# kongzhecn/OMG

Measured on AMD Instinct MI355X. Metric: images/sec @ SDXL 1024^2 50-step, 2-concept mask fusion, higher is better.
Workload: dtype fp16 (storage and MFMA operands; fp32 accumulate; = the reference's own torch_dtype, inference_lora.py:153-159).  Measured tolerance per UNet forward at full size vs the fp32 oracle: rms 1.09e-3, max 4.9e-3 of O(1) outputs — the reference's own fp16 eager execution, emulated op by op in the oracle

## Files before the change

### omg_amd/csrc/misc.hip

```cpp
#include "common.h"
#include <string.h>

static thread_local char g_err[256] = "";
void omg_set_error(const char* msg) { strncpy(g_err, msg ? msg : "", sizeof(g_err) - 1); g_err[sizeof(g_err) - 1] = 0; }
extern "C" const char* omg_last_error(void) { return g_err; }
extern "C" int omg_abi_version(void) { return OMG_ABI_VERSION; }

namespace {

template <typename T, typename TI>
__global__ __launch_bounds__(256) void im2col_in_kernel(const TI* X, int B, int Cin, int H, int W, int KP, char* out) {
  const long npix = (long)B * H * W;
  for (long pix = (long)blockIdx.x * blockDim.x + threadIdx.x; pix < npix; pix += (long)gridDim.x * blockDim.x) {
    const int b = (int)(pix / (H * W)); const int rem = (int)(pix - (long)b * H * W);
    const int y = rem / W, x = rem - y * W;
    for (int c8 = 0; c8 < KP / 8; ++c8) {
      float f[8];
#pragma unroll
      for (int e = 0; e < 8; ++e) {
        const int k = c8 * 8 + e;
        const int tap = k / Cin, ci = k - tap * Cin;
        const int iy = y + tap / 3 - 1, ix = x + tap % 3 - 1;
        const bool ok = (tap < 9) && iy >= 0 && iy < H && ix >= 0 && ix < W;
        f[e] = ok ? (float)X[(((long)b * Cin + ci) * H + iy) * W + ix] : 0.f;
      }
      *(u32x4*)(out + (pix * KP + c8 * 8) * 2) = pack8<T>(f);
    }
  }
}

template <typename T>
__global__ __launch_bounds__(256) void conv_out_kernel(const char* X, int B, int H, int W, int Cin, const char* Wt,
                                                        const T* bias, int Cout, float* Y) {
  const int lane = threadIdx.x & 63, w = threadIdx.x >> 6;
  const long npix = (long)B * H * W;
  const int nvec = Cin / 8;
  const int K = 9 * Cin;
  for (long pix = (long)blockIdx.x * 4 + w; pix < npix; pix += (long)gridDim.x * 4) {
    const int b = (int)(pix / (H * W)); const int rem = (int)(pix - (long)b * H * W);
    const int y = rem / W, x = rem - y * W;
    float acc[8];
#pragma unroll
    for (int e = 0; e < 8; ++e) acc[e] = 0.f;
    for (int i = lane; i < 9 * nvec; i += 64) {
      const int tap = i / nvec, vec = i - tap * nvec;
      const int iy = y + tap / 3 - 1, ix = x + tap % 3 - 1;
      if (iy < 0 || iy >= H || ix < 0 || ix >= W) continue;
      float f[8];
      load8<T>(X + ((((long)b * H + iy) * W + ix) * Cin + vec * 8) * (long)sizeof(T), f);
#pragma unroll
      for (int co = 0; co < 8; ++co) {
        if (co < Cout) {
          float wv[8];
          load8<T>(Wt + ((long)co * K + tap * Cin + vec * 8) * (long)sizeof(T), wv);
#pragma unroll
          for (int e = 0; e < 8; ++e) acc[co] += f[e] * wv[e];
        }
      }
    }
#pragma unroll
    for (int co = 0; co < 8; ++co) {
#pragma unroll
      for (int off = 32; off > 0; off >>= 1) acc[co] += __shfl_xor(acc[co], off);
    }
    if (lane < Cout) {
      float v = 0.f;
#pragma unroll
      for (int co = 0; co < 8; ++co) if (co == lane) v = acc[co];
      Y[(((long)b * Cout + lane) * H + y) * W + x] = v + (bias ? (float)bias[lane] : 0.f);
    }
  }
}

template <typename T> struct Dot2;
template <> struct Dot2<f16> {
  typedef _Float16 v2 __attribute__((ext_vector_type(2)));
  static OMG_DEV float run(unsigned a, unsigned b, float c) { return __builtin_amdgcn_fdot2(__builtin_bit_cast(v2, a), __builtin_bit_cast(v2, b), c, false); }
};
template <> struct Dot2<bf16> {
  typedef __bf16 v2 __attribute__((ext_vector_type(2)));
  static OMG_DEV float run(unsigned a, unsigned b, float c) { return __builtin_amdgcn_fdot2_f32_bf16(__builtin_bit_cast(v2, a), __builtin_bit_cast(v2, b), c, false); }
};
template <typename T, int CO>
__global__ __launch_bounds__(256) void conv_out_pixel_kernel(const char* X, int B, int H, int W, int Cin, const char* Wt, const T* bias, float* Y) {
  const long npix = (long)B * H * W;
  const long pix = (long)blockIdx.x * 256 + threadIdx.x;
  const bool live = pix < npix;
  const long pc = live ? pix : npix - 1;
  const int b = (int)(pc / (H * W)); const int rem = (int)(pc - (long)b * H * W);
  const int y = rem / W, x = rem - y * W;
  const int nvec = Cin / 8;
  const long K2 = 9L * Cin * 2;
  float acc[CO];
#pragma unroll
  for (int co = 0; co < CO; ++co) acc[co] = 0.f;
  for (int tap = 0; tap < 9; ++tap) {
    const int iy = y + tap / 3 - 1, ix = x + tap % 3 - 1;
    const bool ok = ((unsigned)iy < (unsigned)H) & ((unsigned)ix < (unsigned)W);
    const u32x4* px = (const u32x4*)(X + ((((long)b * H + (ok ? iy : y)) * W + (ok ? ix : x)) * Cin) * 2);
    const char* wt = Wt + (long)tap * Cin * 2;
    for (int v0 = 0; v0 < nvec; v0 += 4) {
      u32x4 xv[4];
#pragma unroll
      for (int u = 0; u < 4; ++u) xv[u] = px[v0 + u];
#pragma unroll
      for (int u = 0; u < 4; ++u) {
        if (!ok) xv[u] = u32x4{0u, 0u, 0u, 0u};
#pragma unroll
        for (int co = 0; co < CO; ++co) {
          const u32x4 wv = *(const u32x4*)(wt + co * K2 + (v0 + u) * 16);
#pragma unroll
          for (int j = 0; j < 4; ++j) acc[co] = Dot2<T>::run(xv[u][j], wv[j], acc[co]);
        }
      }
    }
  }
  if (live) {
#pragma unroll
    for (int co = 0; co < CO; ++co) Y[(((long)b * CO + co) * H + y) * W + x] = acc[co] + (bias ? (float)bias[co] : 0.f);
  }
}

template <typename T>
__global__ void timestep_embedding_kernel(const float* t, int n, int dim, T* out, long ldo) {
  const int i = blockIdx.x;
  const int half = dim / 2;
  for (int j = threadIdx.x; j < dim; j += blockDim.x) {
    const int jj = j < half ? j : j - half;
    const float freq = expf(-9.210340371976184f * (float)jj / (float)half);
    const float a = t[i] * freq;
    out[(long)i * ldo + j] = (T)(j < half ? cosf(a) : sinf(a));
  }
}

template <typename T>
__global__ void silu_kernel(const T* x, T* y, long n) {
  for (long i = (long)blockIdx.x * blockDim.x + threadIdx.x; i < n; i += (long)gridDim.x * blockDim.x) y[i] = (T)silu_f((float)x[i]);
}

template <typename T>
__global__ void add_inplace_kernel(char* y, const char* a, long nvec) {
  for (long i = (long)blockIdx.x * blockDim.x + threadIdx.x; i < nvec; i += (long)gridDim.x * blockDim.x) {
    float f[8], g[8];
    unpack8<T>(*(const u32x4*)(y + i * 16), f);
    unpack8<T>(*(const u32x4*)(a + i * 16), g);
#pragma unroll
    for (int e = 0; e < 8; ++e) f[e] += g[e];
    *(u32x4*)(y + i * 16) = pack8<T>(f);
  }
}

template <typename T>
__global__ void copy2d_kernel(const T* src, long lds_, T* dst, long ldd, long rows, long cols) {
  const long n = rows * cols;
  for (long i = (long)blockIdx.x * blockDim.x + threadIdx.x; i < n; i += (long)gridDim.x * blockDim.x) {
    const long r = i / cols, c = i - r * cols;
    dst[r * ldd + c] = src[r * lds_ + c];
  }
}

__global__ void gather_step_kernel(const uint16_t* table, const int* step_idx, uint16_t* out, long n) {
  const long base = (long)(*step_idx) * n;
  for (long i = (long)blockIdx.x * blockDim.x + threadIdx.x; i < n; i += (long)gridDim.x * blockDim.x) out[i] = table[base + i];
}

struct StepP {
  int C, H, W, Hm, Wm, n_concepts, fuse;
  float gs;
  const float* noise;
  const float* region[OMG_MAX_CONCEPTS];
  const float* masks[OMG_MAX_CONCEPTS];
  const float* coef; int* step_idx; int advance;
  float* latents; int out_dtype; void* mi_next; float* fused_out;
};

__global__ __launch_bounds__(256) void step_kernel(StepP p) {
  const int HW = p.H * p.W;
  const int n = p.C * HW;
  const int step = *p.step_idx;
  const float cx = p.coef[step * 4 + 0], ce = p.coef[step * 4 + 1], cin = p.coef[step * 4 + 2];
  for (int i = blockIdx.x * blockDim.x + threadIdx.x; i < n; i += gridDim.x * blockDim.x) {
    const int c = i / HW; const int pix = i - c * HW;
    const int y = pix / p.W, x = pix - y * p.W;
    float unc0 = p.noise[0 * n + i], unc1 = p.noise[1 * n + i];
    float cnd0 = p.noise[2 * n + i], cnd1 = p.noise[3 * n + i];
    if (p.fuse) {
      const int my = (int)(((long)y * p.Hm) / p.H), mx = (int)(((long)x * p.Wm) / p.W);
      bool any = false;
      float add_u = 0.f, add_c = 0.f;
      for (int k = 0; k < p.n_concepts; ++k) {
        if (p.masks[k] == nullptr) continue;
        const bool on = p.masks[k][(long)my * p.Wm + mx] == 1.0f;
        if (on) {
          any = true;
          if (p.region[k]) { add_u += p.region[k][i]; add_c += p.region[k][n + i]; }
        }
      }
      unc1 = (any ? 0.f : unc1) + add_u;
      cnd1 = (any ? 0.f : cnd1) + add_c;
      if (p.fused_out) { p.fused_out[i] = unc1; p.fused_out[n + i] = cnd1; }
    }
    const float e0 = __fmaf_rn(p.gs, __fsub_rn(cnd0, unc0), unc0);
    const float e1 = __fmaf_rn(p.gs, __fsub_rn(cnd1, unc1), unc1);
    const float l0 = __fmaf_rn(ce, e0, __fmul_rn(cx, p.latents[i]));
    const float l1 = __fmaf_rn(ce, e1, __fmul_rn(cx, p.latents[n + i]));
    p.latents[i] = l0; p.latents[n + i] = l1;
    if (p.mi_next) {
      const float a0 = __fmul_rn(l0, cin), a1 = __fmul_rn(l1, cin);
      if (p.out_dtype == OMG_F16) {
        f16* o = (f16*)p.mi_next;
        o[i] = (f16)a0; o[n + i] = (f16)a1; o[2 * n + i] = (f16)a0; o[3 * n + i] = (f16)a1;
      } else if (p.out_dtype == OMG_BF16) {
        bf16* o = (bf16*)p.mi_next;
        o[i] = (bf16)a0; o[n + i] = (bf16)a1; o[2 * n + i] = (bf16)a0; o[3 * n + i] = (bf16)a1;
      } else {
        float* o = (float*)p.mi_next;
        o[i] = a0; o[n + i] = a1; o[2 * n + i] = a0; o[3 * n + i] = a1;
      }
    }
  }
}

__device__ __forceinline__ void step_fuse(const StepP& p, int i, int n, int HW, float& unc1, float& cnd1) {
  const int c = i / HW; const int pix = i - c * HW;
  const int y = pix / p.W, x = pix - y * p.W;
  const int my = (int)(((long)y * p.Hm) / p.H), mx = (int)(((long)x * p.Wm) / p.W);
  bool any = false;
  float add_u = 0.f, add_c = 0.f;
  for (int k = 0; k < p.n_concepts; ++k) {
    if (p.masks[k] == nullptr) continue;
    const bool on = p.masks[k][(long)my * p.Wm + mx] == 1.0f;
    if (on) {
      any = true;
      if (p.region[k]) { add_u += p.region[k][i]; add_c += p.region[k][n + i]; }
    }
  }
  unc1 = (any ? 0.f : unc1) + add_u;
  cnd1 = (any ? 0.f : cnd1) + add_c;
  if (p.fused_out) { p.fused_out[i] = unc1; p.fused_out[n + i] = cnd1; }
}

__device__ __forceinline__ void step_store_input(const StepP& p, int i, int n, float l0, float l1, float cin) {
  const float a0 = __fmul_rn(l0, cin), a1 = __fmul_rn(l1, cin);
  if (p.out_dtype == OMG_F16) {
    f16* o = (f16*)p.mi_next;
    o[i] = (f16)a0; o[n + i] = (f16)a1; o[2 * n + i] = (f16)a0; o[3 * n + i] = (f16)a1;
  } else if (p.out_dtype == OMG_BF16) {
    bf16* o = (bf16*)p.mi_next;
    o[i] = (bf16)a0; o[n + i] = (bf16)a1; o[2 * n + i] = (bf16)a0; o[3 * n + i] = (bf16)a1;
  } else {
    float* o = (float*)p.mi_next;
    o[i] = a0; o[n + i] = a1; o[2 * n + i] = a0; o[3 * n + i] = a1;
  }
}

__global__ __launch_bounds__(256) void step_ms_kernel(StepP p, const float* ms, float* hist) {
  const int HW = p.H * p.W;
  const int n = p.C * HW;
  const float* row = ms + (long)(*p.step_idx) * 8;
  const float a = row[0], b = row[1], cx = row[2], cm = row[3], cp = row[4], cin = row[5];
  const bool use_prev = cp != 0.f;
  for (int i = blockIdx.x * blockDim.x + threadIdx.x; i < n; i += gridDim.x * blockDim.x) {
    float unc0 = p.noise[0 * n + i], unc1 = p.noise[1 * n + i];
    float cnd0 = p.noise[2 * n + i], cnd1 = p.noise[3 * n + i];
    if (p.fuse) step_fuse(p, i, n, HW, unc1, cnd1);
    const float e0 = __fmaf_rn(p.gs, __fsub_rn(cnd0, unc0), unc0);
    const float e1 = __fmaf_rn(p.gs, __fsub_rn(cnd1, unc1), unc1);
    const float x0 = p.latents[i], x1 = p.latents[n + i];
    const float m0 = __fmaf_rn(b, e0, __fmul_rn(a, x0));
    const float m1 = __fmaf_rn(b, e1, __fmul_rn(a, x1));
    float l0 = __fmaf_rn(cm, m0, __fmul_rn(cx, x0));
    float l1 = __fmaf_rn(cm, m1, __fmul_rn(cx, x1));
    if (use_prev) {
      l0 = __fmaf_rn(cp, hist[i], l0);
      l1 = __fmaf_rn(cp, hist[n + i], l1);
    }
    hist[i] = m0; hist[n + i] = m1;
    p.latents[i] = l0; p.latents[n + i] = l1;
    if (p.mi_next) step_store_input(p, i, n, l0, l1, cin);
  }
}

__global__ __launch_bounds__(256) void step_noise_kernel(StepP p, const float* z, long zs) {
  const int HW = p.H * p.W;
  const int n = p.C * HW;
  const int step = *p.step_idx;
  const float cx = p.coef[step * 4 + 0], ce = p.coef[step * 4 + 1], cin = p.coef[step * 4 + 2], cz = p.coef[step * 4 + 3];
  const float* zt = z + (long)step * zs;
  const bool use_z = cz != 0.f;
  for (int i = blockIdx.x * blockDim.x + threadIdx.x; i < n; i += gridDim.x * blockDim.x) {
    float unc0 = p.noise[0 * n + i], unc1 = p.noise[1 * n + i];
    float cnd0 = p.noise[2 * n + i], cnd1 = p.noise[3 * n + i];
    if (p.fuse) step_fuse(p, i, n, HW, unc1, cnd1);
    const float e0 = __fmaf_rn(p.gs, __fsub_rn(cnd0, unc0), unc0);
    const float e1 = __fmaf_rn(p.gs, __fsub_rn(cnd1, unc1), unc1);
    float l0 = __fmaf_rn(ce, e0, __fmul_rn(cx, p.latents[i]));
    float l1 = __fmaf_rn(ce, e1, __fmul_rn(cx, p.latents[n + i]));
    if (use_z) {
      l0 = __fmaf_rn(cz, zt[i], l0);
      l1 = __fmaf_rn(cz, zt[n + i], l1);
    }
    p.latents[i] = l0; p.latents[n + i] = l1;
    if (p.mi_next) step_store_input(p, i, n, l0, l1, cin);
  }
}

__global__ void step_advance_kernel(int* step_idx) { *step_idx = *step_idx + 1; }

__global__ void scale_model_input_kernel(const float* latents, const float* cin, int n, int out_dtype, void* out) {
  const float c = *cin;
  for (int i = blockIdx.x * blockDim.x + threadIdx.x; i < 2 * n; i += gridDim.x * blockDim.x) {
    const float v = latents[i] * c;
    if (out_dtype == OMG_F16) { ((f16*)out)[i] = (f16)v; ((f16*)out)[2 * n + i] = (f16)v; }
    else if (out_dtype == OMG_BF16) { ((bf16*)out)[i] = (bf16)v; ((bf16*)out)[2 * n + i] = (bf16)v; }
    else { ((float*)out)[i] = v; ((float*)out)[2 * n + i] = v; }
  }
}

}

extern "C" int omg_conv_in(int dtype, const void* X, int x_is_f32, int B, int Cin, int H, int W, const void* Wt,
                           const void* bias, int Cout, void* workspace, void* Y, void* stream) {
  OMG_REQUIRE(dtype == OMG_F16 || dtype == OMG_BF16, "omg_conv_in: dtype");
  OMG_REQUIRE(X && Wt && Y && workspace && Cout % 8 == 0 && Cin > 0 && 9 * Cin <= 64, "omg_conv_in: args (9*Cin <= 64)");
  const long npix = (long)B * H * W;
  if (npix == 0) return OMG_OK;
  const int KP = 64;
  long blocks = (npix + 255) / 256; if (blocks > 8192) blocks = 8192;
  hipStream_t s = (hipStream_t)stream;
  if (dtype == OMG_F16) {
    if (x_is_f32) OMG_LAUNCH((im2col_in_kernel<f16, float>), dim3(blocks), dim3(256), 0, s, (const float*)X, B, Cin, H, W, KP, (char*)workspace);
    else OMG_LAUNCH((im2col_in_kernel<f16, f16>), dim3(blocks), dim3(256), 0, s, (const f16*)X, B, Cin, H, W, KP, (char*)workspace);
  } else {
    if (x_is_f32) OMG_LAUNCH((im2col_in_kernel<bf16, float>), dim3(blocks), dim3(256), 0, s, (const float*)X, B, Cin, H, W, KP, (char*)workspace);
    else OMG_LAUNCH((im2col_in_kernel<bf16, bf16>), dim3(blocks), dim3(256), 0, s, (const bf16*)X, B, Cin, H, W, KP, (char*)workspace);
  }
  int rc = omg_check_launch("im2col_in");
  if (rc) return rc;
  omg_gemm_args g{};
  g.dtype = dtype; g.M = (int)npix; g.N = Cout; g.K = KP;
  g.A = workspace; g.lda = KP; g.W = Wt; g.ldw = KP;
  g.groups = 1; g.rows_per_group = (int)npix; g.bias = bias; g.act = OMG_ACT_NONE; g.out_scale = 1.0f;
  g.C = Y; g.ldc = Cout;
  return omg_gemm(&g, stream);
}

template <typename T>
__global__ __launch_bounds__(256) void cast_f32_kernel(const char* X, float* Y, long n8) {
  for (long i = (long)blockIdx.x * 256 + threadIdx.x; i < n8; i += (long)gridDim.x * 256) {
    float f[8];
    load8<T>(X + i * 16, f);
    store8<float>((char*)(Y + i * 8), f);
  }
}

extern "C" int omg_cast_f32(int dtype, const void* X, float* Y, int64_t n, void* stream) {
  OMG_REQUIRE(dtype == OMG_F16 || dtype == OMG_BF16, "omg_cast_f32: dtype");
  OMG_REQUIRE(X && Y && n % 8 == 0, "omg_cast_f32: args");
  if (n == 0) return OMG_OK;
  long blocks = (n / 8 + 255) / 256; if (blocks > 16384) blocks = 16384;
  hipStream_t s = (hipStream_t)stream;
  if (dtype == OMG_F16) OMG_LAUNCH(cast_f32_kernel<f16>, dim3(blocks), dim3(256), 0, s, (const char*)X, Y, (long)(n / 8));
  else OMG_LAUNCH(cast_f32_kernel<bf16>, dim3(blocks), dim3(256), 0, s, (const char*)X, Y, (long)(n / 8));
  return omg_check_launch("cast_f32");
}

extern "C" int omg_conv_out(int dtype, const void* X, int B, int H, int W, int Cin, const void* Wt, const void* bias,
                            int Cout, float* Y, void* stream) {
  OMG_REQUIRE(dtype == OMG_F16 || dtype == OMG_BF16 || dtype == OMG_F32, "omg_conv_out: dtype");
  OMG_REQUIRE(X && Wt && Y && Cin % 8 == 0 && Cout >= 1 && Cout <= 8, "omg_conv_out: args");
  const long npix = (long)B * H * W;
  if (npix == 0) return OMG_OK;
  long blocks = (npix + 3) / 4; if (blocks > 8192) blocks = 8192;
  hipStream_t s = (hipStream_t)stream;
  if (dtype != OMG_F32 && Cout == 4 && Cin % 32 == 0 && (((uintptr_t)X | (uintptr_t)Wt) & 15) == 0) {
    const unsigned pb = (unsigned)((npix + 255) / 256);
    if (dtype == OMG_F16) OMG_LAUNCH((conv_out_pixel_kernel<f16, 4>), dim3(pb), dim3(256), 0, s, (const char*)X, B, H, W, Cin, (const char*)Wt, (const f16*)bias, Y);
    else OMG_LAUNCH((conv_out_pixel_kernel<bf16, 4>), dim3(pb), dim3(256), 0, s, (const char*)X, B, H, W, Cin, (const char*)Wt, (const bf16*)bias, Y);
    return omg_check_launch("conv_out_pixel");
  }
  if (dtype == OMG_F16) OMG_LAUNCH(conv_out_kernel<f16>, dim3(blocks), dim3(256), 0, s, (const char*)X, B, H, W, Cin, (const char*)Wt, (const f16*)bias, Cout, Y);
  else if (dtype == OMG_BF16) OMG_LAUNCH(conv_out_kernel<bf16>, dim3(blocks), dim3(256), 0, s, (const char*)X, B, H, W, Cin, (const char*)Wt, (const bf16*)bias, Cout, Y);
  else OMG_LAUNCH(conv_out_kernel<float>, dim3(blocks), dim3(256), 0, s, (const char*)X, B, H, W, Cin, (const char*)Wt, (const float*)bias, Cout, Y);
  return omg_check_launch("conv_out");
}

extern "C" int omg_timestep_embedding(int dtype, const float* t, int n, int dim, void* out, int64_t ldo, void* stream) {
  OMG_REQUIRE(dtype == OMG_F16 || dtype == OMG_BF16, "omg_timestep_embedding: dtype");
  OMG_REQUIRE(t && out && dim % 2 == 0 && n >= 0, "omg_timestep_embedding: args");
  if (n == 0) return OMG_OK;
  hipStream_t s = (hipStream_t)stream;
  if (dtype == OMG_F16) OMG_LAUNCH(timestep_embedding_kernel<f16>, dim3(n), dim3(128), 0, s, t, n, dim, (f16*)out, (long)ldo);
  else OMG_LAUNCH(timestep_embedding_kernel<bf16>, dim3(n), dim3(128), 0, s, t, n, dim, (bf16*)out, (long)ldo);
  return omg_check_launch("timestep_embedding");
}

template <typename T>
__global__ __launch_bounds__(256) void softmax_rows_kernel(T* X, long cols, long ld, float scale) {
  __shared__ float red[8];
  T* row = X + (long)blockIdx.x * ld;
  const int tid = threadIdx.x, lane = tid & 63, w = tid >> 6;
  float m = -3.0e38f;
  for (long c = tid; c < cols; c += 256) m = fmaxf(m, (float)row[c]);
  for (int o = 32; o > 0; o >>= 1) m = fmaxf(m, __shfl_xor(m, o));
  if (lane == 0) red[w] = m;
  __syncthreads();
  m = fmaxf(fmaxf(red[0], red[1]), fmaxf(red[2], red[3])) * scale;
  const float sl2 = scale * 1.4426950408889634f, ml2 = m * 1.4426950408889634f;
  float sum = 0.f;
  for (long c = tid; c < cols; c += 256) sum += __builtin_amdgcn_exp2f((float)row[c] * sl2 - ml2);
  for (int o = 32; o > 0; o >>= 1) sum += __shfl_xor(sum, o);
  if (lane == 0) red[4 + w] = sum;
  __syncthreads();
  const float inv = 1.0f / (red[4] + red[5] + red[6] + red[7]);
  for (long c = tid; c < cols; c += 256) row[c] = (T)(__builtin_amdgcn_exp2f((float)row[c] * sl2 - ml2) * inv);
}

__global__ __launch_bounds__(256) void channel_mix_kernel(const float* X, const float* Wm, const float* bias, int Cin, int Cout,
                                                          long HW, float* Y) {
  const int b = blockIdx.y;
  for (long p = (long)blockIdx.x * 256 + threadIdx.x; p < HW; p += (long)gridDim.x * 256) {
    float x[8];
    for (int c = 0; c < Cin; ++c) x[c] = X[((long)b * Cin + c) * HW + p];
    for (int o = 0; o < Cout; ++o) {
      float a = bias ? bias[o] : 0.f;
      for (int c = 0; c < Cin; ++c) a = __fmaf_rn(Wm[o * Cin + c], x[c], a);
      Y[((long)b * Cout + o) * HW + p] = a;
    }
  }
}

extern "C" int omg_softmax_rows(int dtype, void* X, int64_t rows, int64_t cols, int64_t ld, float scale, void* stream) {
  OMG_REQUIRE(dtype == OMG_F16 || dtype == OMG_BF16, "omg_softmax_rows: dtype");
  OMG_REQUIRE(X && rows >= 0 && cols > 0 && ld >= cols && rows < 2147483647L, "omg_softmax_rows: args");
  if (rows == 0) return OMG_OK;
  hipStream_t s = (hipStream_t)stream;
  if (dtype == OMG_F16) OMG_LAUNCH(softmax_rows_kernel<f16>, dim3((unsigned)rows), dim3(256), 0, s, (f16*)X, (long)cols, (long)ld, scale);
  else OMG_LAUNCH(softmax_rows_kernel<bf16>, dim3((unsigned)rows), dim3(256), 0, s, (bf16*)X, (long)cols, (long)ld, scale);
  return omg_check_launch("softmax_rows");
}

extern "C" int omg_channel_mix(const float* X, const float* Wm, const float* bias, int B, int Cin, int Cout, int64_t HW,
                               float* Y, void* stream) {
  OMG_REQUIRE(X && Wm && Y && B >= 0 && HW > 0, "omg_channel_mix: args");
  OMG_REQUIRE(Cin >= 1 && Cin <= 8 && Cout >= 1 && Cout <= 8, "omg_channel_mix: 1 <= Cin, Cout <= 8");
  if (B == 0) return OMG_OK;
  long blocks = (HW + 255) / 256;
  if (blocks > 1024) blocks = 1024;
  OMG_LAUNCH(channel_mix_kernel, dim3((unsigned)blocks, (unsigned)B), dim3(256), 0, (hipStream_t)stream, X, Wm, bias, Cin, Cout, (long)HW, Y);
  return omg_check_launch("channel_mix");
}

extern "C" int omg_silu(int dtype, const void* x, void* y, int64_t n, void* stream) {
  OMG_REQUIRE(dtype == OMG_F16 || dtype == OMG_BF16, "omg_silu: dtype");
  OMG_REQUIRE(x && y, "omg_silu: null");
  if (n == 0) return OMG_OK;
  long blocks = (n + 255) / 256; if (blocks > 2048) blocks = 2048;
  hipStream_t s = (hipStream_t)stream;
  if (dtype == OMG_F16) OMG_LAUNCH(silu_kernel<f16>, dim3(blocks), dim3(256), 0, s, (const f16*)x, (f16*)y, (long)n);
  else OMG_LAUNCH(silu_kernel<bf16>, dim3(blocks), dim3(256), 0, s, (const bf16*)x, (bf16*)y, (long)n);
  return omg_check_launch("silu");
}

extern "C" int omg_add_inplace(int dtype, void* y, const void* a, int64_t n, void* stream) {
  OMG_REQUIRE(dtype == OMG_F16 || dtype == OMG_BF16, "omg_add_inplace: dtype");
  OMG_REQUIRE(y && a && n % 8 == 0, "omg_add_inplace: n % 8");
  if (n == 0) return OMG_OK;
  const long nvec = n / 8;
  long blocks = (nvec + 255) / 256; if (blocks > 4096) blocks = 4096;
  hipStream_t s = (hipStream_t)stream;
  if (dtype == OMG_F16) OMG_LAUNCH(add_inplace_kernel<f16>, dim3(blocks), dim3(256), 0, s, (char*)y, (const char*)a, nvec);
  else OMG_LAUNCH(add_inplace_kernel<bf16>, dim3(blocks), dim3(256), 0, s, (char*)y, (const char*)a, nvec);
  return omg_check_launch("add_inplace");
}

extern "C" int omg_copy2d(int dtype, const void* src, int64_t lds_, void* dst, int64_t ldd, int64_t rows, int64_t cols, void* stream) {
  OMG_REQUIRE(dtype == OMG_F16 || dtype == OMG_BF16, "omg_copy2d: dtype");
  OMG_REQUIRE(src && dst, "omg_copy2d: null");
  const long n = rows * cols;
  if (n == 0) return OMG_OK;
  long blocks = (n + 255) / 256; if (blocks > 2048) blocks = 2048;
  hipStream_t s = (hipStream_t)stream;
  OMG_LAUNCH(copy2d_kernel<uint16_t>, dim3(blocks), dim3(256), 0, s, (const uint16_t*)src, (long)lds_, (uint16_t*)dst, (long)ldd, (long)rows, (long)cols);
  return omg_check_launch("copy2d");
}

extern "C" int omg_gather_step(int dtype, const void* table, const int32_t* step_idx, void* out, int64_t n_per_step, void* stream) {
  OMG_REQUIRE(dtype == OMG_F16 || dtype == OMG_BF16, "omg_gather_step: dtype");
  OMG_REQUIRE(table && step_idx && out && n_per_step > 0, "omg_gather_step: args");
  long blocks = (n_per_step + 255) / 256; if (blocks > 1024) blocks = 1024;
  OMG_LAUNCH(gather_step_kernel, dim3(blocks), dim3(256), 0, (hipStream_t)stream, (const uint16_t*)table, (const int*)step_idx, (uint16_t*)out, (long)n_per_step);
  return omg_check_launch("gather_step");
}

static StepP step_params(const omg_step_args* a) {
  StepP p{};
  p.C = a->C; p.H = a->H; p.W = a->W; p.Hm = a->Hm; p.Wm = a->Wm; p.n_concepts = a->n_concepts; p.fuse = a->fuse;
  p.gs = a->guidance_scale; p.noise = a->noise_pred;
  for (int k = 0; k < OMG_MAX_CONCEPTS; ++k) { p.region[k] = k < a->n_concepts ? a->region_pred[k] : nullptr; p.masks[k] = k < a->n_concepts ? a->masks[k] : nullptr; }
  p.coef = a->coef; p.step_idx = a->step_idx; p.advance = a->advance;
  p.latents = a->latents; p.out_dtype = a->out_dtype; p.mi_next = a->model_input_next; p.fused_out = a->fused_noise_out;
  return p;
}

extern "C" int omg_fuse_cfg_step(const omg_step_args* a, void* stream) {
  OMG_REQUIRE(a != nullptr, "omg_fuse_cfg_step: null args");
  OMG_REQUIRE(a->noise_pred && a->coef && a->step_idx && a->latents, "omg_fuse_cfg_step: null operand");
  OMG_REQUIRE(a->n_concepts >= 0 && a->n_concepts <= OMG_MAX_CONCEPTS, "omg_fuse_cfg_step: n_concepts");
  OMG_REQUIRE(a->C > 0 && a->H > 0 && a->W > 0, "omg_fuse_cfg_step: shape");
  if (a->fuse) OMG_REQUIRE(a->Hm > 0 && a->Wm > 0, "omg_fuse_cfg_step: mask shape");
  const StepP p = step_params(a);
  const int n = a->C * a->H * a->W;
  int blocks = (n + 255) / 256; if (blocks > 1024) blocks = 1024;
  hipStream_t s = (hipStream_t)stream;
  OMG_LAUNCH(step_kernel, dim3(blocks), dim3(256), 0, s, p);
  if (a->advance) OMG_LAUNCH(step_advance_kernel, dim3(1), dim3(1), 0, s, a->step_idx);
  return omg_check_launch("fuse_cfg_step");
}

extern "C" int omg_fuse_cfg_step_ms(const omg_step_args* a, const float* ms_coef, float* x0_hist, void* stream) {
  OMG_REQUIRE(a != nullptr, "omg_fuse_cfg_step_ms: null args");
  OMG_REQUIRE(a->noise_pred && a->step_idx && a->latents && ms_coef && x0_hist, "omg_fuse_cfg_step_ms: null operand");
  OMG_REQUIRE(a->n_concepts >= 0 && a->n_concepts <= OMG_MAX_CONCEPTS, "omg_fuse_cfg_step_ms: n_concepts");
  OMG_REQUIRE(a->C > 0 && a->H > 0 && a->W > 0, "omg_fuse_cfg_step_ms: shape");
  if (a->fuse) OMG_REQUIRE(a->Hm > 0 && a->Wm > 0, "omg_fuse_cfg_step_ms: mask shape");
  const StepP p = step_params(a);
  const int n = a->C * a->H * a->W;
  int blocks = (n + 255) / 256; if (blocks > 1024) blocks = 1024;
  hipStream_t s = (hipStream_t)stream;
  OMG_LAUNCH(step_ms_kernel, dim3(blocks), dim3(256), 0, s, p, ms_coef, x0_hist);
  if (a->advance) OMG_LAUNCH(step_advance_kernel, dim3(1), dim3(1), 0, s, a->step_idx);
  return omg_check_launch("fuse_cfg_step_ms");
}

extern "C" int omg_fuse_cfg_step_noise(const omg_step_args* a, const float* z, int64_t z_step_stride, void* stream) {
  OMG_REQUIRE(a != nullptr, "omg_fuse_cfg_step_noise: null args");
  OMG_REQUIRE(a->noise_pred && a->coef && a->step_idx && a->latents && z, "omg_fuse_cfg_step_noise: null operand");
  OMG_REQUIRE(a->n_concepts >= 0 && a->n_concepts <= OMG_MAX_CONCEPTS, "omg_fuse_cfg_step_noise: n_concepts");
  OMG_REQUIRE(a->C > 0 && a->H > 0 && a->W > 0, "omg_fuse_cfg_step_noise: shape");
  OMG_REQUIRE(z_step_stride >= 2L * a->C * a->H * a->W, "omg_fuse_cfg_step_noise: z_step_stride");
  if (a->fuse) OMG_REQUIRE(a->Hm > 0 && a->Wm > 0, "omg_fuse_cfg_step_noise: mask shape");
  const StepP p = step_params(a);
  const int n = a->C * a->H * a->W;
  int blocks = (n + 255) / 256; if (blocks > 1024) blocks = 1024;
  hipStream_t s = (hipStream_t)stream;
  OMG_LAUNCH(step_noise_kernel, dim3(blocks), dim3(256), 0, s, p, z, (long)z_step_stride);
  if (a->advance) OMG_LAUNCH(step_advance_kernel, dim3(1), dim3(1), 0, s, a->step_idx);
  return omg_check_launch("fuse_cfg_step_noise");
}

extern "C" int omg_scale_model_input(int dtype, const float* latents, const float* coef_cin, int n_per_sample, void* out, void* stream) {
  OMG_REQUIRE(latents && coef_cin && out, "omg_scale_model_input: null");
  OMG_REQUIRE(dtype == OMG_F16 || dtype == OMG_BF16 || dtype == 2, "omg_scale_model_input: dtype");
  int blocks = (2 * n_per_sample + 255) / 256; if (blocks > 1024) blocks = 1024;
  OMG_LAUNCH(scale_model_input_kernel, dim3(blocks), dim3(256), 0, (hipStream_t)stream, latents, coef_cin, n_per_sample, dtype, out);
  return omg_check_launch("scale_model_input");
}
```

### omg_amd/unet.py

```python
from __future__ import annotations

from dataclasses import dataclass
from types import SimpleNamespace
from typing import Dict, List, Optional, Sequence, Tuple

import torch
from torch import nn

from . import _lib as L
from . import ops
from ._checkpoint import PackedCache
from .attention import Attention, FusedAttnProcessor
from .modules import Conv2d, GEGLU, GroupNorm, LayerNorm, Linear, LoraState, bump_pointer_epoch, bump_weights_version


@dataclass
class UNetConfig:
    in_channels: int = 4
    out_channels: int = 4
    sample_size: int = 128
    block_out_channels: Tuple[int, ...] = (320, 640, 1280)
    down_block_types: Tuple[str, ...] = ("DownBlock2D", "CrossAttnDownBlock2D", "CrossAttnDownBlock2D")
    up_block_types: Tuple[str, ...] = ("CrossAttnUpBlock2D", "CrossAttnUpBlock2D", "UpBlock2D")
    layers_per_block: int = 2
    transformer_layers_per_block: Tuple[int, ...] = (1, 2, 10)
    attention_head_dim: Tuple[int, ...] = (5, 10, 20)
    cross_attention_dim: int = 2048
    addition_time_embed_dim: int = 256
    projection_class_embeddings_input_dim: int = 2816
    norm_num_groups: int = 32
    norm_eps: float = 1e-5
    time_cond_proj_dim: Optional[int] = None

    @staticmethod
    def sdxl() -> "UNetConfig":
        return UNetConfig()

    @staticmethod
    def tiny() -> "UNetConfig":
        return UNetConfig(sample_size=16, block_out_channels=(64, 128, 256), transformer_layers_per_block=(1, 1, 2),
                          attention_head_dim=(1, 2, 4), cross_attention_dim=128, addition_time_embed_dim=32,
                          projection_class_embeddings_input_dim=64 + 6 * 32)


class _Ctx:

    __slots__ = ("silu_emb", "ehs", "B")

    def __init__(self, silu_emb, ehs, B):
        self.silu_emb, self.ehs, self.B = silu_emb, ehs, B


class TimestepEmbedding(nn.Module):
    def __init__(self, cin, dim, dtype, device):
        super().__init__()
        self.linear_1 = Linear(cin, dim, dtype=dtype, device=device)
        self.linear_2 = Linear(dim, dim, dtype=dtype, device=device)

    def forward(self, x, residual=None):
        return self.linear_2(self.linear_1(x, act=L.ACT_SILU), residual=residual)


class ResnetBlock2D(nn.Module):
    def __init__(self, cin, cout, temb_dim, groups, eps, dtype, device):
        super().__init__()
        self.norm1 = GroupNorm(groups, cin, eps, dtype, device)
        self.conv1 = Conv2d(cin, cout, 3, dtype=dtype, device=device)
        self.time_emb_proj = Linear(temb_dim, cout, dtype=dtype, device=device)
        self.norm2 = GroupNorm(groups, cout, eps, dtype, device)
        self.conv2 = Conv2d(cout, cout, 3, dtype=dtype, device=device)
        self.conv_shortcut = Conv2d(cin, cout, 1, dtype=dtype, device=device) if cin != cout else None

    def forward(self, x, ctx: _Ctx, x2=None):
        h = self.norm1(x, x2=x2, silu=True, mx8=self.conv1.mx8_ok())
        tproj = self.time_emb_proj(ctx.silu_emb)
        h = self.conv1(h, group_bias=tproj)
        h = self.norm2(h, silu=True, mx8=self.conv2.mx8_ok())
        if self.conv_shortcut is not None:
            sc = self.conv_shortcut(x, x2=x2)
        else:
            if x2 is not None:
                raise L.OmgHipError("concat input without a shortcut conv cannot happen in the SDXL topology")
            sc = x
        return self.conv2(h, residual=sc)


class FeedForward(nn.Module):
    def __init__(self, dim, dtype, device):
        super().__init__()
        self.net = nn.ModuleList([GEGLU(dim, dim * 4, dtype, device), nn.Identity(), Linear(dim * 4, dim, dtype=dtype, device=device)])

    def forward(self, x, residual=None):
        return self.net[2](self.net[0](x, out_mx8=self.net[2].mx8 and self.net[2]._mx8_ok()), residual=residual)


class BasicTransformerBlock(nn.Module):
    def __init__(self, dim, heads, cross_dim, dtype, device):
        super().__init__()
        self.norm1 = LayerNorm(dim, dtype=dtype, device=device)
        self.attn1 = Attention(dim, None, heads, dtype=dtype, device=device)
        self.norm2 = LayerNorm(dim, dtype=dtype, device=device)
        self.attn2 = Attention(dim, cross_dim, heads, dtype=dtype, device=device)
        self.norm3 = LayerNorm(dim, dtype=dtype, device=device)
        self.ff = FeedForward(dim, dtype, device)

    @staticmethod
    def _attend(attn, x, h, ehs, kw):
        if getattr(attn.processor, "supports_fused_residual", False):
            return attn(x, encoder_hidden_states=ehs, residual=h, **kw)
        return attn(x, encoder_hidden_states=ehs, **kw) + h

    def forward(self, h, ehs, kw):
        fused = getattr(self.attn1.processor, "supports_fused_residual", False) and getattr(self.attn2.processor, "supports_fused_residual", False)
        h = self._attend(self.attn1, self.norm1(h, mx8=fused and self.attn1.to_q.mx8 and not self.attn1._has_lora()), h, None, kw)
        h = self._attend(self.attn2, self.norm2(h, mx8=fused and self.attn2.to_q.mx8 and self.attn2.to_q._mx8_ok()), h, ehs, kw)
        return self.ff(self.norm3(h, mx8=self.ff.net[0].proj.mx8 and self.ff.net[0].proj._mx8_ok()), residual=h)


class Transformer2DModel(nn.Module):
    def __init__(self, dim, heads, layers, cross_dim, groups, dtype, device):
        super().__init__()
        self.norm = GroupNorm(groups, dim, 1e-6, dtype, device)
        self.proj_in = Linear(dim, dim, dtype=dtype, device=device)
        self.transformer_blocks = nn.ModuleList([BasicTransformerBlock(dim, heads, cross_dim, dtype, device) for _ in range(layers)])
        self.proj_out = Linear(dim, dim, dtype=dtype, device=device)

    def forward(self, x, ehs, kw):
        B, H, W, C = x.shape
        h = self.proj_in(self.norm(x).view(B, H * W, C))
        for blk in self.transformer_blocks:
            h = blk(h, ehs, kw)
        return self.proj_out(h, residual=x.view(B, H * W, C)).view(B, H, W, C)


class Downsample2D(nn.Module):
    def __init__(self, c, dtype, device):
        super().__init__()
        self.conv = Conv2d(c, c, 3, stride=2, dtype=dtype, device=device)

    def forward(self, x):
        return self.conv(x)


class Upsample2D(nn.Module):
    def __init__(self, c, dtype, device):
        super().__init__()
        self.conv = Conv2d(c, c, 3, dtype=dtype, device=device)
        self.conv.upsamples = True

    def forward(self, x):
        return self.conv(x, upsample=True)


class _DownBlock(nn.Module):
    def __init__(self, cfg, i, cin, cout, has_attn, add_down, dtype, device):
        super().__init__()
        ted = cfg.block_out_channels[0] * 4
        self.resnets = nn.ModuleList([ResnetBlock2D(cin if j == 0 else cout, cout, ted, cfg.norm_num_groups, cfg.norm_eps, dtype, device)
                                      for j in range(cfg.layers_per_block)])
        if has_attn:
            self.attentions = nn.ModuleList([Transformer2DModel(cout, cfg.attention_head_dim[i], cfg.transformer_layers_per_block[i],
                                                                cfg.cross_attention_dim, cfg.norm_num_groups, dtype, device)
                                             for _ in range(cfg.layers_per_block)])
        self.has_attn = has_attn
        self.downsamplers = nn.ModuleList([Downsample2D(cout, dtype, device)]) if add_down else None

    def forward(self, h, ctx, kw, skips):
        for j, res in enumerate(self.resnets):
            h = res(h, ctx)
            if self.has_attn:
                h = self.attentions[j](h, ctx.ehs, kw)
            skips.append(h)
        if self.downsamplers is not None:
            h = self.downsamplers[0](h)
            skips.append(h)
        return h


class DownBlock2D(_DownBlock):
    pass


class CrossAttnDownBlock2D(_DownBlock):
    pass


class UNetMidBlock2DCrossAttn(nn.Module):
    def __init__(self, cfg, dtype, device):
        super().__init__()
        c = cfg.block_out_channels[-1]
        ted = cfg.block_out_channels[0] * 4
        self.resnets = nn.ModuleList([ResnetBlock2D(c, c, ted, cfg.norm_num_groups, cfg.norm_eps, dtype, device) for _ in range(2)])
        self.attentions = nn.ModuleList([Transformer2DModel(c, cfg.attention_head_dim[-1], cfg.transformer_layers_per_block[-1],
                                                            cfg.cross_attention_dim, cfg.norm_num_groups, dtype, device)])

    def forward(self, h, ctx, kw):
        h = self.resnets[0](h, ctx)
        h = self.attentions[0](h, ctx.ehs, kw)
        return self.resnets[1](h, ctx)


class _UpBlock(nn.Module):
    def __init__(self, cfg, heads, layers, prev_c, cout, in_c, has_attn, add_up, dtype, device):
        super().__init__()
        ted = cfg.block_out_channels[0] * 4
        n = cfg.layers_per_block + 1
        self.resnets = nn.ModuleList()
        for j in range(n):
            skip = in_c if j == n - 1 else cout
            rin = prev_c if j == 0 else cout
            self.resnets.append(ResnetBlock2D(rin + skip, cout, ted, cfg.norm_num_groups, cfg.norm_eps, dtype, device))
        if has_attn:
            self.attentions = nn.ModuleList([Transformer2DModel(cout, heads, layers, cfg.cross_attention_dim, cfg.norm_num_groups, dtype, device)
                                             for _ in range(n)])
        self.has_attn = has_attn
        self.upsamplers = nn.ModuleList([Upsample2D(cout, dtype, device)]) if add_up else None

    def forward(self, h, ctx, kw, skips):
        for j, res in enumerate(self.resnets):
            h = res(h, ctx, x2=skips.pop())
            if self.has_attn:
                h = self.attentions[j](h, ctx.ehs, kw)
        if self.upsamplers is not None:
            h = self.upsamplers[0](h)
        return h


class UpBlock2D(_UpBlock):
    pass


class CrossAttnUpBlock2D(_UpBlock):
    pass


MX8_CLASSES = ("qkv", "attn_out", "cross_q", "cross_out", "geglu", "ff_out", "proj_in", "proj_out", "conv1", "conv2")
MX8_PRESETS = {"all": MX8_CLASSES, "safe": ("cross_q", "cross_out", "ff_out"), "none": ()}


def mx8_class_of(name: str, module) -> Optional[str]:
    if isinstance(module, Linear) and ".attentions." in name:
        for suffix, cls in ((".attn1.to_q", "qkv"), (".attn1.to_k", "qkv"), (".attn1.to_v", "qkv"), (".attn1.to_out.0", "attn_out"),
                            (".attn2.to_q", "cross_q"), (".attn2.to_out.0", "cross_out"), (".ff.net.0.proj", "geglu"), (".ff.net.2", "ff_out"),
                            (".proj_in", "proj_in"), (".proj_out", "proj_out")):
            if name.endswith(suffix):
                return cls if module.in_features % 128 == 0 else None
        return None
    if isinstance(module, Conv2d) and ".resnets." in name and (name.endswith(".conv1") or name.endswith(".conv2")):
        return name[-5:]
    return None


def set_mx8_classes(net, classes, select=None) -> int:
    if isinstance(classes, str):
        classes = MX8_PRESETS.get(classes, (classes,))
    classes = set(classes or ())
    unknown = classes - set(MX8_CLASSES)
    if unknown:
        raise ValueError(f"unknown MX-fp8 layer classes {sorted(unknown)}; known: {MX8_CLASSES}")
    changed, n_on = False, 0
    for name, m in net.named_modules():
        if not isinstance(m, (Linear, Conv2d)):
            continue
        cls = mx8_class_of(name, m)
        new = cls is not None and cls in classes and (select is None or bool(select(name, cls)))
        changed |= bool(getattr(m, "mx8", False)) != new
        m.mx8 = new
        n_on += int(new)
    if changed:
        bump_pointer_epoch()
        bump_weights_version(net)
    return n_on


class UNet2DConditionModel(PackedCache):
    def __init__(self, config: Optional[UNetConfig] = None, dtype: torch.dtype = torch.float16, device=None):
        super().__init__()
        cfg = config or UNetConfig.sdxl()
        self.config = cfg
        self._dtype = dtype
        c0 = cfg.block_out_channels[0]
        ted = c0 * 4
        if cfg.time_cond_proj_dim is not None:
            raise L.OmgHipError("time_cond_proj_dim (LCM guidance embedding) is not part of SDXL-base")
        self.conv_in = Conv2d(cfg.in_channels, c0, 3, dtype=dtype, device=device)
        self.time_embedding = TimestepEmbedding(c0, ted, dtype, device)
        self.add_embedding = TimestepEmbedding(cfg.projection_class_embeddings_input_dim, ted, dtype, device)
        nb = len(cfg.block_out_channels)
        self.down_blocks = nn.ModuleList()
        self.up_blocks = nn.ModuleList()
        cout = c0
        for i, typ in enumerate(cfg.down_block_types):
            cin, cout = cout, cfg.block_out_channels[i]
            cls = CrossAttnDownBlock2D if typ == "CrossAttnDownBlock2D" else DownBlock2D
            self.down_blocks.append(cls(cfg, i, cin, cout, typ == "CrossAttnDownBlock2D", i != nb - 1, dtype, device))
        self.mid_block = UNetMidBlock2DCrossAttn(cfg, dtype, device)
        rev = list(reversed(cfg.block_out_channels))
        rev_heads = list(reversed(cfg.attention_head_dim))
        rev_layers = list(reversed(cfg.transformer_layers_per_block))
        cout = rev[0]
        for i, typ in enumerate(cfg.up_block_types):
            prev_c, cout = cout, rev[i]
            in_c = rev[min(i + 1, nb - 1)]
            cls = CrossAttnUpBlock2D if typ == "CrossAttnUpBlock2D" else UpBlock2D
            self.up_blocks.append(cls(cfg, rev_heads[i], rev_layers[i], prev_c, cout, in_c, typ == "CrossAttnUpBlock2D", i != nb - 1, dtype, device))
        self.conv_norm_out = GroupNorm(cfg.norm_num_groups, c0, cfg.norm_eps, dtype, device)
        self.conv_out = Conv2d(c0, cfg.out_channels, 3, dtype=dtype, device=device)
        self._lora_modules: Optional[List[nn.Module]] = None

    @property
    def dtype(self):
        return self._dtype

    @property
    def device(self):
        return self.conv_in.weight.device

    def attentions(self):
        for name, m in self.named_modules():
            if isinstance(m, Attention):
                yield name, m

    @property
    def attn_processors(self) -> Dict[str, object]:
        return {f"{name}.processor": m.processor for name, m in self.attentions()}

    def set_attn_processor(self, processor) -> None:
        if isinstance(processor, dict):
            for name, m in self.attentions():
                m.set_processor(processor[f"{name}.processor"])
        else:
            for _, m in self.attentions():
                m.set_processor(processor)

    def set_default_attn_processor(self) -> None:
        self.set_attn_processor(FusedAttnProcessor())

    def invalidate_packed(self) -> None:
        super().invalidate_packed()
        for m in self.modules():
            if m is not self and hasattr(m, "invalidate_packed"):
                m.invalidate_packed()

    def _load_from_state_dict(self, *a, **k):
        bump_weights_version(self)
        return super()._load_from_state_dict(*a, **k)

    def init_synthetic_(self, seed: int = 0, qk_gain: float = 1.0) -> "UNet2DConditionModel":
        g = torch.Generator(device=self.device).manual_seed(seed)
        for name, p in self.named_parameters():
            if name.endswith(".weight") and p.dim() >= 2:
                fan_in = p[0].numel()
                w = torch.randn(p.shape, generator=g, device=p.device, dtype=torch.float32) * fan_in ** -0.5
                if ".to_q." in name or ".to_k." in name:
                    w *= qk_gain
            elif name.endswith(".weight"):
                w = 1.0 + 0.1 * torch.randn(p.shape, generator=g, device=p.device, dtype=torch.float32)
            else:
                w = 0.1 * torch.randn(p.shape, generator=g, device=p.device, dtype=torch.float32)
            p.data.copy_(w.to(p.dtype))
        self.invalidate_packed()
        return self

    def set_linear_precision(self, mode: str = "fp16") -> None:
        if mode not in ("fp16", "mx8"):
            raise ValueError(mode)
        on = mode == "mx8"
        changed = False
        for name, m in self.named_modules():
            if isinstance(m, Linear):
                in_block = ".attentions." in name and not (name.endswith(".to_k") or name.endswith(".to_v")) or \
                           (".attentions." in name and ".attn1." in name)
                new = on and in_block and m.in_features % 128 == 0
                changed |= bool(getattr(m, "mx8", False)) != new
                m.mx8 = new
        self.linear_precision = mode
        if changed:
            bump_pointer_epoch()
            bump_weights_version(self)

    def set_conv_precision(self, mode: str = "fp16") -> None:
        if mode not in ("fp16", "mx8"):
            raise ValueError(mode)
        changed = False
        for m in self.modules():
            if isinstance(m, ResnetBlock2D):
                changed |= bool(getattr(m.conv1, "mx8", False)) != (mode == "mx8")
                m.conv1.mx8 = m.conv2.mx8 = mode == "mx8"
        self.conv_precision = mode
        if changed:
            bump_pointer_epoch()
            bump_weights_version(self)

    def set_precision_classes(self, classes, select=None) -> int:
        if isinstance(classes, str):
            classes = MX8_PRESETS.get(classes, (classes,))
        n = set_mx8_classes(self, classes, select)
        cl = set(classes or ())
        self.linear_precision = "mx8" if cl - {"conv1", "conv2"} else "fp16"
        self.conv_precision = "mx8" if cl & {"conv1", "conv2"} else "fp16"
        return n

    def set_lora_state(self, state: Optional[LoraState]) -> None:
        if self._lora_modules is None:
            self._lora_modules = [m for m in self.modules() if isinstance(m, (Linear, Conv2d))]
        for m in self._lora_modules:
            m.lora_state = state

    def refresh_cross_kv(self, ctx: torch.Tensor, state: Optional[LoraState]) -> None:
        self.set_lora_state(state)
        try:
            for _, m in self.attentions():
                if m.is_cross:
                    m.project_cross(ctx)
        finally:
            self.set_lora_state(None)

    def refresh_ip_kv(self, ip_ctx: torch.Tensor) -> None:
        from .attention import _ip_kv
        for _, m in self.attentions():
            if m.is_cross and getattr(m, "ip_kv_weight", None) is not None:
                _ip_kv(m, ip_ctx)

    def _pack(self):
        return {"in": ops.pack_conv_in_weight(self.conv_in.weight.data), "out": self.conv_out.weight.data.permute(0, 2, 3, 1).contiguous()}

    @staticmethod
    def _nhwc(r: torch.Tensor, dt) -> torch.Tensor:
        v = r.permute(0, 2, 3, 1)
        if v.dtype != dt:
            v = v.to(dt)
        return v if v.is_contiguous() else v.contiguous()

    def time_embed(self, timestep, B: int, text_embeds: torch.Tensor, time_ids: torch.Tensor) -> torch.Tensor:
        cfg = self.config
        dev, dt = self.device, self._dtype
        if not torch.is_tensor(timestep):
            t = torch.full((B,), float(timestep), dtype=torch.float32, device=dev)
        else:
            t = timestep.to(device=dev, dtype=torch.float32).reshape(-1)
            if t.numel() == 1:
                t = t.expand(B).contiguous()
        t_emb = ops.timestep_embedding(t.contiguous(), cfg.block_out_channels[0], dt)
        te_dim = text_embeds.shape[-1]
        add = torch.empty((B, cfg.projection_class_embeddings_input_dim), dtype=dt, device=dev)
        ops.copy2d(text_embeds.to(dt).contiguous(), add[:, :te_dim])
        tid = time_ids.to(device=dev, dtype=torch.float32).reshape(-1).contiguous()
        n_ids = tid.numel() // B
        tmp = ops.timestep_embedding(tid, cfg.addition_time_embed_dim, dt)
        ops.copy2d(tmp.view(B, n_ids * cfg.addition_time_embed_dim), add[:, te_dim:])
        aug = self.add_embedding(add)
        return self.time_embedding(t_emb, residual=aug)

    def forward(self, sample: torch.Tensor, timestep, encoder_hidden_states: torch.Tensor, class_labels=None,
                timestep_cond=None, attention_mask=None, cross_attention_kwargs=None, added_cond_kwargs=None,
                down_block_additional_residuals: Optional[Sequence[torch.Tensor]] = None,
                mid_block_additional_residual: Optional[torch.Tensor] = None, encoder_attention_mask=None,
                return_dict: bool = False, emb: Optional[torch.Tensor] = None, out: Optional[torch.Tensor] = None):
        if attention_mask is not None or encoder_attention_mask is not None or class_labels is not None or timestep_cond is not None:
            raise L.OmgHipError("attention_mask / class_labels / timestep_cond are not used on OMG's SDXL path")
        if not sample.is_cuda:
            raise L.OmgHipError("UNet2DConditionModel runs on the MI355X only (no CPU fallback)")
        cfg = self.config
        B, _, H, W = sample.shape
        dt = self._dtype
        kw = dict(cross_attention_kwargs or {})
        kw.pop("scale", None)
        row_residuals = kw.pop("omg_residuals", None)
        if emb is None:
            if added_cond_kwargs is None:
                raise L.OmgHipError("added_cond_kwargs={'text_embeds','time_ids'} is required (addition_embed_type='text_time')")
            emb = self.time_embed(timestep, B, added_cond_kwargs["text_embeds"], added_cond_kwargs["time_ids"])
        ctx = _Ctx(ops.silu(emb), encoder_hidden_states.to(dt).contiguous() if encoder_hidden_states.dtype != dt or not encoder_hidden_states.is_contiguous() else encoder_hidden_states, B)
        bw = self._pk()
        x_in = sample.contiguous()
        if x_in.dtype not in (torch.float32, dt):
            x_in = x_in.to(dt)
        h = ops.conv_in(x_in, bw["in"], self.conv_in.bias, dt)
        skips: List[torch.Tensor] = [h]
        for blk in self.down_blocks:
            h = blk(h, ctx, kw, skips)
        if down_block_additional_residuals is not None:
            if len(down_block_additional_residuals) != len(skips):
                raise ValueError(f"expected {len(skips)} down-block residuals, got {len(down_block_additional_residuals)}")
            skips[-1] = skips[-1].clone()
            for s_, r in zip(skips, down_block_additional_residuals):
                ops.add_(s_, self._nhwc(r, dt))
        if row_residuals:
            skips[-1] = skips[-1].clone() if down_block_additional_residuals is None else skips[-1]
            for r0, r1, down, _ in row_residuals:
                for s_, r in zip(skips, down):
                    ops.add_(s_[r0:r1], self._nhwc(r, dt))
        h = self.mid_block(h, ctx, kw)
        if mid_block_additional_residual is not None:
            ops.add_(h, self._nhwc(mid_block_additional_residual, dt))
        if row_residuals:
            for r0, r1, _, mid in row_residuals:
                ops.add_(h[r0:r1], self._nhwc(mid, dt))
        for blk in self.up_blocks:
            h = blk(h, ctx, kw, skips)
        h = self.conv_norm_out(h, silu=True)
        y = ops.conv_out(h, bw["out"], self.conv_out.bias, out=out)
        if out is None and sample.dtype != torch.float32:
            y = y.to(sample.dtype)
        if return_dict:
            return SimpleNamespace(sample=y)
        return (y,)
```

Measured before the change: 0.4340.

## Batch resnet time-embedding projections into one GEMM and add strip-tiled fp32 conv_out

The per-ResnetBlock time_emb_proj linears are concatenated into one weight matrix, so a single GEMM per UNet forward produces all time projections, which are then sliced per block. This falls back to per-block projection when LoRA state is attached. Separately, a new LDS-staged 8x8 strip kernel handles fp32 3x3 convolutions with 3 output channels and Cin up to 168, which looks like the VAE decoder output conv rather than the UNet path. The strip kernel adds dynamic shared memory use and a one-time attribute set.

```diff
diff --git a/omg_amd/csrc/misc.hip b/omg_amd/csrc/misc.hip
--- a/omg_amd/csrc/misc.hip
+++ b/omg_amd/csrc/misc.hip
@@ -118,6 +118,98 @@
   if (live) {
 #pragma unroll
     for (int co = 0; co < CO; ++co) Y[(((long)b * CO + co) * H + y) * W + x] = acc[co] + (bias ? (float)bias[co] : 0.f);
+  }
+}
+
+constexpr int CS_R = 8, CS_S = 8, CS_HALO = (CS_R + 2) * (CS_S + 2);
+inline size_t conv_strip_lds(int Cin, size_t elem) { return (size_t)CS_HALO * (Cin * elem + 16); }
+
+template <int NT, int U>
+OMG_DEV void conv_strip_stage(char* lds, const char* X, int b, int y0, int x0, int H, int W, int rowb, int pitch) {
+  const int nvec = rowb >> 4, total = CS_HALO * nvec;
+  for (int v0 = threadIdx.x; v0 < total; v0 += U * NT) {
+    u32x4 r[U];
+#pragma unroll
+    for (int u = 0; u < U; ++u) {
+      const int v = v0 + u * NT;
+      r[u] = u32x4{0u, 0u, 0u, 0u};
+      if (v < total) {
+        const int hp = v / nvec, cv = v - hp * nvec;
+        const int hy = hp / (CS_S + 2), hx = hp - hy * (CS_S + 2);
+        const int iy = y0 + hy - 1, ix = x0 + hx - 1;
+        if (((unsigned)iy < (unsigned)H) & ((unsigned)ix < (unsigned)W)) r[u] = *(const u32x4*)(X + (((long)b * H + iy) * W + ix) * rowb + cv * 16);
+      }
+    }
+#pragma unroll
+    for (int u = 0; u < U; ++u) {
+      const int v = v0 + u * NT;
+      if (v < total) { const int hp = v / nvec, cv = v - hp * nvec; *(u32x4*)(lds + hp * pitch + cv * 16) = r[u]; }
+    }
+  }
+}
+
+template <int CO, int NI>
+__global__ __launch_bounds__(256) void conv_out_strip_f32_kernel(const char* X, int B, int H, int W, int Cin, const char* Wt, const float* bias, float* Y) {
+  extern __shared__ __attribute__((aligned(16))) char cs_lds[];
+  const int tx = (W + CS_S - 1) / CS_S, ty = (H + CS_R - 1) / CS_R;
+  int blk = blockIdx.x;
+  const int b = blk / (tx * ty); blk -= b * tx * ty;
+  const int y0 = (blk / tx) * CS_R, x0 = (blk % tx) * CS_S;
+  const int rowb = Cin * 4, pitch = rowb + 16;
+  const int lane = threadIdx.x & 63, w = __builtin_amdgcn_readfirstlane(threadIdx.x >> 6);
+  const int nvec = Cin / 8, K = 9 * Cin;
+  float wv[NI][CO][8];
+  int off[NI];
+#pragma unroll
+  for (int k = 0; k < NI; ++k) {
+    const int i = lane + 64 * k;
+    const bool on = i < 9 * nvec;
+    const int tap = on ? i / nvec : 0, vec = on ? i - tap * nvec : 0;
+    off[k] = ((tap / 3) * (CS_S + 2) + tap % 3) * pitch + vec * 32;
+#pragma unroll
+    for (int co = 0; co < CO; ++co) {
+      load8<float>(Wt + ((long)co * K + tap * Cin + vec * 8) * 4L, wv[k][co]);
+      if (!on) {
+#pragma unroll
+        for (int e = 0; e < 8; ++e) wv[k][co][e] = 0.f;
+      }
+    }
+  }
+  conv_strip_stage<256, 8>(cs_lds, X, b, y0, x0, H, W, rowb, pitch);
+  __syncthreads();
+  for (int pp = 0; pp < CS_R * CS_S / 4; ++pp) {
+    const int p = w * (CS_R * CS_S / 4) + pp;
+    const int ly = p / CS_S, lx = p % CS_S;
+    const int y = y0 + ly, x = x0 + lx;
+    if (y >= H || x >= W) continue;
+    const char* base = cs_lds + (ly * (CS_S + 2) + lx) * pitch;
+    float acc[CO];
+#pragma unroll
+    for (int co = 0; co < CO; ++co) acc[co] = 0.f;
+#pragma unroll
+    for (int k = 0; k < NI; ++k) {
+      if (lane + 64 * k < 9 * nvec) {
+        float f[8];
+        load8<float>(base + off[k], f);
+#pragma unroll
+        for (int co = 0; co < CO; ++co) {
+#pragma clang fp contract(off)
+#pragma unroll
+          for (int e = 0; e < 8; ++e) acc[co] += f[e] * wv[k][co][e];
+        }
+      }
+    }
+#pragma unroll
+    for (int co = 0; co < CO; ++co) {
+#pragma unroll
+      for (int o = 32; o > 0; o >>= 1) acc[co] += __shfl_xor(acc[co], o);
+    }
+    if (lane < CO) {
+      float v = 0.f;
+#pragma unroll
+      for (int co = 0; co < CO; ++co) if (co == lane) v = acc[co];
+      Y[(((long)b * CO + lane) * H + y) * W + x] = v + (bias ? (float)bias[lane] : 0.f);
+    }
   }
 }
 
@@ -373,6 +465,14 @@
   if (npix == 0) return OMG_OK;
   long blocks = (npix + 3) / 4; if (blocks > 8192) blocks = 8192;
   hipStream_t s = (hipStream_t)stream;
+  const bool al16 = (((uintptr_t)X | (uintptr_t)Wt) & 15) == 0;
+  const long strips = (long)B * ((H + CS_R - 1) / CS_R) * ((W + CS_S - 1) / CS_S);
+  if (dtype == OMG_F32 && Cout == 3 && Cin <= 168 && al16 && strips <= 0x7fffffffL) {
+    static bool attr_f = false;
+    if (!attr_f) { attr_f = true; (void)hipFuncSetAttribute((const void*)conv_out_strip_f32_kernel<3, 3>, hipFuncAttributeMaxDynamicSharedMemorySize, (int)conv_strip_lds(168, 4)); }
+    OMG_LAUNCH((conv_out_strip_f32_kernel<3, 3>), dim3((unsigned)strips), dim3(256), conv_strip_lds(Cin, 4), s, (const char*)X, B, H, W, Cin, (const char*)Wt, (const float*)bias, Y);
+    return omg_check_launch("conv_out_strip_f32");
+  }
   if (dtype != OMG_F32 && Cout == 4 && Cin % 32 == 0 && (((uintptr_t)X | (uintptr_t)Wt) & 15) == 0) {
     const unsigned pb = (unsigned)((npix + 255) / 256);
     if (dtype == OMG_F16) OMG_LAUNCH((conv_out_pixel_kernel<f16, 4>), dim3(pb), dim3(256), 0, s, (const char*)X, B, H, W, Cin, (const char*)Wt, (const f16*)bias, Y);
diff --git a/omg_amd/unet.py b/omg_amd/unet.py
--- a/omg_amd/unet.py
+++ b/omg_amd/unet.py
@@ -45,10 +45,11 @@
 
 class _Ctx:
 
-    __slots__ = ("silu_emb", "ehs", "B")
-
-    def __init__(self, silu_emb, ehs, B):
+    __slots__ = ("silu_emb", "ehs", "B", "tproj")
+
+    def __init__(self, silu_emb, ehs, B, tproj=None):
         self.silu_emb, self.ehs, self.B = silu_emb, ehs, B
+        self.tproj = tproj
 
 
 class TimestepEmbedding(nn.Module):
@@ -73,7 +74,9 @@
 
     def forward(self, x, ctx: _Ctx, x2=None):
         h = self.norm1(x, x2=x2, silu=True, mx8=self.conv1.mx8_ok())
-        tproj = self.time_emb_proj(ctx.silu_emb)
+        tproj = ctx.tproj.get(self) if ctx.tproj else None
+        if tproj is None:
+            tproj = self.time_emb_proj(ctx.silu_emb)
         h = self.conv1(h, group_bias=tproj)
         h = self.norm2(h, silu=True, mx8=self.conv2.mx8_ok())
         if self.conv_shortcut is not None:
@@ -423,7 +426,24 @@
                 _ip_kv(m, ip_ctx)
 
     def _pack(self):
-        return {"in": ops.pack_conv_in_weight(self.conv_in.weight.data), "out": self.conv_out.weight.data.permute(0, 2, 3, 1).contiguous()}
+        res = [m for m in self.modules() if isinstance(m, ResnetBlock2D)]
+        return {"in": ops.pack_conv_in_weight(self.conv_in.weight.data), "out": self.conv_out.weight.data.permute(0, 2, 3, 1).contiguous(),
+                "temb_res": res, "temb_w": torch.cat([m.time_emb_proj.weight.data for m in res], 0),
+                "temb_b": torch.cat([m.time_emb_proj.bias.data for m in res], 0)}
+
+    def _time_projections(self, bw, silu_emb):
+        res = bw["temb_res"]
+        for m in res:
+            lin = m.time_emb_proj
+            if lin.out_features % 8 != 0 or (lin.lora_state is not None and (lin.w_slots is not None or lin.lora_down is not None)):
+                return None
+        y = ops.gemm(silu_emb, bw["temb_w"], bias=bw["temb_b"])
+        out, c = {}, 0
+        for m in res:
+            n = m.time_emb_proj.out_features
+            out[m] = y[:, c:c + n]
+            c += n
+        return out
 
     @staticmethod
     def _nhwc(r: torch.Tensor, dt) -> torch.Tensor:
@@ -473,6 +493,7 @@
             emb = self.time_embed(timestep, B, added_cond_kwargs["text_embeds"], added_cond_kwargs["time_ids"])
         ctx = _Ctx(ops.silu(emb), encoder_hidden_states.to(dt).contiguous() if encoder_hidden_states.dtype != dt or not encoder_hidden_states.is_contiguous() else encoder_hidden_states, B)
         bw = self._pk()
+        ctx.tproj = self._time_projections(bw, ctx.silu_emb)
         x_in = sample.contiguous()
         if x_in.dtype not in (torch.float32, dt):
             x_in = x_in.to(dt)
```

After: 0.4346, median of 6. No clear change (+0.1%).
